# eldariont/svim-asm

Measured on AMD Instinct MI355X. Metric: CIGAR ops/sec (SV-signature extraction, human genome-genome alignment), higher is better.
Workload: dtype u32

## Files before the change

### svim_asm_amd/csrc/svx_cigar.hip

```cpp
#include "svx_internal.h"
#include "svx_postpass_dev.h"
#include "svx_segments_dev.h"

namespace {

#ifndef SVX_LANE_OPS
#define SVX_LANE_OPS 16
#endif
constexpr int kLaneOps = SVX_LANE_OPS;
constexpr int kLU = kLaneOps / 4;
constexpr int kRoundOps = 64 * kLaneOps;
#ifndef SVX_ROUNDS
#define SVX_ROUNDS 4
#endif
constexpr int kRounds = SVX_ROUNDS;
constexpr int kTileOps = kRoundOps * kRounds;
#ifndef SVX_SLAB
#define SVX_SLAB 128
#endif
constexpr int kSlab = SVX_SLAB;
#ifndef SVX_WAVES
#define SVX_WAVES 4
#endif
constexpr int kWaves = SVX_WAVES;
constexpr int kXposeU4 = 64 * kLU;
constexpr int kScanBlock = 1024;

enum { MODE_STAGE = 0, MODE_DIRECT = 1 };

struct CigarArgs {
    const uint32_t* cigar;
    const uint8_t* op;
    const uint64_t* aln_off;
    uint32_t* tile_alo;
// ... 1454 lines not shown
    a->rows = SegRowArgs{d_cigar, d_aln_off, q.d_seg_src, q.d_seg_tid, q.d_seg_pos, q.d_seg_rev, q.d_seg_qend, q.n_segs,
                         q.d_read_off, q.n_reads, q.d_segs, q.d_read_len};
    a->seg_rl = svx_ws_take<int32_t>(ctx, q.n_segs ? q.n_segs : 1);
    a->tree.segs = q.d_segs;
    a->tree.seg_rl = a->seg_rl;
    a->tree.read_len_out = q.d_read_len;
    a->tree.sorted = svx_ws_take<svx_seg>(ctx, q.n_segs ? q.n_segs : 1);
    a->tree.read_off = q.d_read_off;
    a->tree.read_len = q.d_read_len;
    a->tree.n_reads = q.n_reads;
    a->tree.o = q.params;
    a->tree.out = q.d_raw;
    svx_post_dev::PostArgs& o = a->post;
    o.raw = q.d_raw; o.read_off = q.d_read_off; o.n_reads = q.n_reads; o.contig_rank = q.d_contig_rank; o.n_contigs = q.n_contigs;
    o.min_sv = q.params.min_sv_size; o.max_sv = q.params.max_sv_size;
    o.out = q.d_post; o.out_off = q.d_post_off; o.out_cnt = q.d_post_cnt;
    o.scratch = svx_ws_take<char>(ctx, (size_t)q.n_reads * post_stride);
    o.scratch_off = nullptr;
    o.scratch_stride = post_stride;
#ifndef SVX_A3_READS_DIV
#define SVX_A3_READS_DIV 1024u
#endif
#ifndef SVX_A3_READS_MAX
#define SVX_A3_READS_MAX 32u
#endif
    const uint32_t per = q.n_reads / SVX_A3_READS_DIV;
    const uint32_t least = q.n_reads < 384u ? 1u : 2u;
    a->reads_per_block = per < least ? least : (per > SVX_A3_READS_MAX ? SVX_A3_READS_MAX : per);
    a->deal = q.n_deal_blocks ? q.d_deal : nullptr;
    a->n_deal = q.n_deal_blocks;
}

template <bool SOA>
int cigar_extract_dev_impl(svx_ctx* ctx, const uint32_t* d_cigar_or_len, const uint8_t* d_op,
                           uint64_t n_ops, const uint64_t* d_aln_off, uint32_t n_aln,
                           const int32_t* d_ref_start, uint32_t min_len, svx_sig_soa d_out,
                           uint64_t cap, uint64_t* d_n_out, const svx_a3_plan* a3 = nullptr) {
    if (!ctx || !d_n_out) return SVX_E_INVALID;
    if (n_ops >= (1ull << 32)) {
        SVX_SET_ERR(ctx, "n_ops=%llu exceeds the 2^32-1 per-call limit; split the batch",
                    (unsigned long long)n_ops);
        return SVX_E_TOO_LARGE;
    }
    SVX_HIP(ctx, hipSetDevice(ctx->device));
    if (n_ops == 0 || n_aln == 0) {
        SVX_HIP(ctx, hipMemsetAsync(d_n_out, 0, sizeof(uint64_t), ctx->stream));
        return a3 ? SVX_E_INVALID : SVX_OK;
    }
    if (!d_cigar_or_len || !d_aln_off || (SOA && !d_op)) return SVX_E_INVALID;
    if (cap > 0 && (!d_out.aln || !d_out.ref_pos || !d_out.read_pos || !d_out.len || !d_out.type))
        return SVX_E_INVALID;
    if ((reinterpret_cast<uintptr_t>(d_cigar_or_len) & 15u) ||
        (SOA && (reinterpret_cast<uintptr_t>(d_op) & 15u))) {
        SVX_SET_ERR(ctx, "device CIGAR buffers must be 16-byte aligned");
        return SVX_E_INVALID;
    }
    const bool small = n_ops <= (uint64_t)kSmallMaxTiles * kSmallTileOps && n_ops <= ctx->small_batch_ops;
    const uint32_t n_tiles = small ? (uint32_t)((n_ops + kSmallTileOps - 1) / kSmallTileOps)
                                   : (uint32_t)((n_ops + kTileOps - 1) / kTileOps);
    size_t need = svx_cigar_extract_ws_need(ctx, n_ops);
    if (a3) need += svx_take_bytes(a3->n_segs ? a3->n_segs : 1, sizeof(svx_seg)) + svx_take_bytes(a3->n_segs ? a3->n_segs : 1, 4) +
                    svx_take_bytes((size_t)a3->n_reads * a3->post_stride, 1);
    int rc = svx_ws_reserve(ctx, need);
    if (rc != SVX_OK) return rc;

    CigarArgs a;
    a.cigar = d_cigar_or_len;
    a.op = d_op;
    a.aln_off = d_aln_off;
    a.ref_start = d_ref_start;
    a.n_ops = n_ops;
    a.n_aln = n_aln;
    a.n_tiles = n_tiles;
    a.min_len = min_len;
    a.n_dense = reinterpret_cast<uint32_t*>(ctx->ws);
    a.desc = svx_ws_take<uint4>(ctx, n_tiles);
    a.desc4 = svx_ws_take<uint4>(ctx, (n_tiles + kWaves - 1) / kWaves);
    a.slab = svx_ws_take<uint4>(ctx, (size_t)n_tiles * kSlab);
    a.out_base = svx_ws_take<uint32_t>(ctx, n_tiles);
    a.carry_ref = svx_ws_take<uint32_t>(ctx, n_tiles);
    a.carry_read = svx_ws_take<uint32_t>(ctx, n_tiles);
    a.dense_list = svx_ws_take<uint32_t>(ctx, n_tiles);
    a.tile_alo = svx_ws_take<uint32_t>(ctx, n_tiles);
    const uint32_t n_scan_blocks = (n_tiles + kScanBlock - 1) / kScanBlock;
    a.blk_agg = svx_ws_take<uint4>(ctx, n_scan_blocks);
    a.blk_prefix = svx_ws_take<uint4>(ctx, n_scan_blocks);
    a.out = d_out;
    a.cap = cap;
    A3Args c;
    memset(&c, 0, sizeof(c));
    uint32_t n_a3_blocks = 0, n_post_blocks = 0;
    if (a3) {
        a3_fill(ctx, d_cigar_or_len, d_aln_off, *a3, a3->post_stride, &c);
        n_a3_blocks = c.deal ? c.n_deal : (a3->n_reads + c.reads_per_block - 1) / c.reads_per_block;
        n_post_blocks = (a3->n_reads + 255u) / 256u;
    }

    if (small) {
        rc = svx_timing_begin(ctx);
        if (rc != SVX_OK) return rc;
        rc = svx_timing_mark(ctx, 1);
        if (rc != SVX_OK) return rc;
        const uint32_t tile_blocks = (n_tiles + kWaves - 1) / kWaves;
        if (a3)
            hipLaunchKernelGGL((k_tiles_a3<SOA, kSmallTileOps, ALO_SEARCH>), dim3(n_a3_blocks + tile_blocks), dim3(64 * kWaves), 0,
                               ctx->stream, a, c, n_a3_blocks);
        else
            hipLaunchKernelGGL((k_cigar_tiles<SOA, kSmallTileOps, ALO_SEARCH>), dim3(tile_blocks), dim3(64 * kWaves), 0,
                               ctx->stream, a);
        rc = svx_timing_mark(ctx, 2);
        if (rc != SVX_OK) return rc;
        if (ctx->want_dom) {
            if (!ctx->ev_dom) SVX_HIP(ctx, hipEventCreateWithFlags(&ctx->ev_dom, hipEventDisableTiming));
            SVX_HIP(ctx, hipEventRecord(ctx->ev_dom, ctx->stream));
            ctx->ev_dom_recorded = true;
        }
#ifndef SVX_FIN_MIN_BLOCKS
#define SVX_FIN_MIN_BLOCKS 128u
#endif
        uint32_t fin_blocks = (n_tiles + kFinTiles - 1) / kFinTiles;
        if (fin_blocks < SVX_FIN_MIN_BLOCKS) fin_blocks = SVX_FIN_MIN_BLOCKS;
        if (a3)
            hipLaunchKernelGGL((k_cigar_finish_small<SOA, true>), dim3(n_post_blocks + fin_blocks), dim3(256), 0, ctx->stream, a, d_n_out,
                               c, n_post_blocks);
        else
            hipLaunchKernelGGL((k_cigar_finish_small<SOA, false>), dim3(fin_blocks), dim3(256), 0, ctx->stream, a, d_n_out, c, 0u);
        SVX_HIP(ctx, hipGetLastError());
        return svx_timing_end(ctx);
    }
    const uint32_t blocks_all = (n_tiles + kWaves - 1) / kWaves;
    const uint32_t blocks_cap = (uint32_t)ctx->n_cu * 8u;
    const uint32_t finish_blocks = (n_tiles + 256 / kFinLanes - 1) / (256 / kFinLanes);
    const uint32_t dense_blocks = n_tiles < blocks_cap ? n_tiles : blocks_cap;
    rc = svx_timing_begin(ctx);
    if (rc != SVX_OK) return rc;
    hipLaunchKernelGGL(k_tile_alo, dim3((n_aln + 255) / 256), dim3(256), 0, ctx->stream, d_aln_off, n_aln, n_tiles,
                       a.tile_alo);
    rc = svx_timing_mark(ctx, 1);
    if (rc != SVX_OK) return rc;
    hipLaunchKernelGGL((k_cigar_tiles<SOA, kTileOps, ALO_TABLE>), dim3(blocks_all), dim3(64 * kWaves), 0, ctx->stream, a);
    rc = svx_timing_mark(ctx, 2);
    if (rc != SVX_OK) return rc;
    if (ctx->want_dom) {
        if (!ctx->ev_dom) SVX_HIP(ctx, hipEventCreateWithFlags(&ctx->ev_dom, hipEventDisableTiming));
        SVX_HIP(ctx, hipEventRecord(ctx->ev_dom, ctx->stream));
        ctx->ev_dom_recorded = true;
    }
    hipLaunchKernelGGL(k_desc_scan, dim3(n_scan_blocks), dim3(kScanBlock), 0, ctx->stream, a.desc, n_tiles,
                       a.out_base, a.carry_ref, a.carry_read, a.dense_list, a.n_dense, a.blk_agg,
                       a.blk_prefix, a.n_dense + 1, d_n_out);
    if (a3) {
        hipLaunchKernelGGL(k_finish_a3, dim3(n_a3_blocks + finish_blocks), dim3(256), 0, ctx->stream, a, c, n_a3_blocks);
        hipLaunchKernelGGL((k_cigar_dense<SOA, true>), dim3(n_post_blocks + dense_blocks), dim3(64 * kWaves), 0, ctx->stream, a, c,
                           n_post_blocks);
    } else {
        hipLaunchKernelGGL(k_cigar_finish, dim3(finish_blocks), dim3(256), 0, ctx->stream, a);
        hipLaunchKernelGGL((k_cigar_dense<SOA, false>), dim3(dense_blocks), dim3(64 * kWaves), 0, ctx->stream, a, c, 0u);
    }
    SVX_HIP(ctx, hipGetLastError());
    return svx_timing_end(ctx);
}

int validate_offsets(svx_ctx* ctx, const uint64_t* aln_off, uint32_t n_aln) {
    if (n_aln == 0) return SVX_OK;
    if (!aln_off) return SVX_E_INVALID;
    if (aln_off[0] != 0) {
        SVX_SET_ERR(ctx, "aln_off[0] must be 0");
        return SVX_E_INVALID;
    }
    for (uint32_t i = 0; i < n_aln; ++i)
        if (aln_off[i + 1] < aln_off[i]) {
            SVX_SET_ERR(ctx, "aln_off must be non-decreasing (index %u)", i);
            return SVX_E_INVALID;
        }
    return SVX_OK;
}

template <bool SOA>
int cigar_extract_host_impl(svx_ctx* ctx, const uint32_t* cigar_or_len, const uint8_t* op,
                            const uint64_t* aln_off, uint32_t n_aln, const int32_t* ref_start,
                            uint32_t min_len, svx_sig_soa out, uint64_t cap, uint64_t* n_out) {
    if (!ctx || !n_out) return SVX_E_INVALID;
    *n_out = 0;
    int rc = validate_offsets(ctx, aln_off, n_aln);
    if (rc != SVX_OK) return rc;
    const uint64_t n_ops = n_aln ? aln_off[n_aln] : 0;
    if (n_ops == 0) return SVX_OK;
    if (!cigar_or_len || (SOA && !op)) return SVX_E_INVALID;
    if (n_ops >= (1ull << 32)) return SVX_E_TOO_LARGE;
    SVX_HIP(ctx, hipSetDevice(ctx->device));
    size_t need = svx_take_bytes(n_ops, 4) + (SOA ? svx_take_bytes(n_ops, 1) : 0) +
// ... 30 lines not shown
    if (m) {
        SVX_HIP(ctx, hipMemcpyAsync(out.aln, d_out.aln, m * 4, hipMemcpyDeviceToHost, ctx->stream));
        SVX_HIP(ctx, hipMemcpyAsync(out.ref_pos, d_out.ref_pos, m * 4, hipMemcpyDeviceToHost, ctx->stream));
        SVX_HIP(ctx, hipMemcpyAsync(out.read_pos, d_out.read_pos, m * 4, hipMemcpyDeviceToHost, ctx->stream));
        SVX_HIP(ctx, hipMemcpyAsync(out.len, d_out.len, m * 4, hipMemcpyDeviceToHost, ctx->stream));
        SVX_HIP(ctx, hipMemcpyAsync(out.type, d_out.type, m, hipMemcpyDeviceToHost, ctx->stream));
        SVX_HIP(ctx, hipStreamSynchronize(ctx->stream));
    }
    if (n > cap) {
        SVX_SET_ERR(ctx, "output capacity %llu < %llu signatures", (unsigned long long)cap,
                    (unsigned long long)n);
        return SVX_E_CAPACITY;
    }
    return SVX_OK;
}

}

extern "C" int svx_cigar_extract_dev(svx_ctx* ctx, const uint32_t* d_cigar, uint64_t n_ops,
                                     const uint64_t* d_aln_off, uint32_t n_aln,
                                     const int32_t* d_ref_start, uint32_t min_len, svx_sig_soa d_out,
                                     uint64_t cap, uint64_t* d_n_out) {
    return cigar_extract_dev_impl<false>(ctx, d_cigar, nullptr, n_ops, d_aln_off, n_aln, d_ref_start,
                                         min_len, d_out, cap, d_n_out);
}

int svx_cigar_extract_chain_dev(svx_ctx* ctx, const uint32_t* d_cigar, uint64_t n_ops, const uint64_t* d_aln_off, uint32_t n_aln,
                                const int32_t* d_ref_start, uint32_t min_len, svx_sig_soa d_out, uint64_t cap,
                                uint64_t* d_n_out, const svx_a3_plan* a3) {
    return cigar_extract_dev_impl<false>(ctx, d_cigar, nullptr, n_ops, d_aln_off, n_aln, d_ref_start, min_len, d_out, cap,
                                         d_n_out, a3);
}

extern "C" int svx_cigar_extract_soa_dev(svx_ctx* ctx, const uint8_t* d_op, const uint32_t* d_len,
                                         uint64_t n_ops, const uint64_t* d_aln_off, uint32_t n_aln,
                                         const int32_t* d_ref_start, uint32_t min_len,
                                         svx_sig_soa d_out, uint64_t cap, uint64_t* d_n_out) {
    return cigar_extract_dev_impl<true>(ctx, d_len, d_op, n_ops, d_aln_off, n_aln, d_ref_start,
                                        min_len, d_out, cap, d_n_out);
}

extern "C" int svx_cigar_extract(svx_ctx* ctx, const uint32_t* cigar, const uint64_t* aln_off,
                                 uint32_t n_aln, const int32_t* ref_start, uint32_t min_len,
                                 svx_sig_soa out, uint64_t cap, uint64_t* n_out) {
    return cigar_extract_host_impl<false>(ctx, cigar, nullptr, aln_off, n_aln, ref_start, min_len,
                                          out, cap, n_out);
}

extern "C" int svx_cigar_extract_soa(svx_ctx* ctx, const uint8_t* op, const uint32_t* len,
                                     const uint64_t* aln_off, uint32_t n_aln,
                                     const int32_t* ref_start, uint32_t min_len, svx_sig_soa out,
                                     uint64_t cap, uint64_t* n_out) {
    return cigar_extract_host_impl<true>(ctx, len, op, aln_off, n_aln, ref_start, min_len, out, cap,
                                         n_out);
}

extern "C" int svx_cigar_stats_dev(svx_ctx* ctx, const uint32_t* d_cigar, uint64_t n_ops,
                                   const uint64_t* d_aln_off, uint32_t n_aln, svx_aln_stats d_out) {
    if (!ctx) return SVX_E_INVALID;
    if (n_aln == 0) return SVX_OK;
    if (!d_aln_off || (n_ops && !d_cigar)) return SVX_E_INVALID;
    SVX_HIP(ctx, hipSetDevice(ctx->device));
    StatsArgs a{d_cigar, d_aln_off, n_aln, d_out};
    uint32_t blocks = (n_aln + 3) / 4;
    uint32_t cap = (uint32_t)ctx->n_cu * 8u;
    hipLaunchKernelGGL(k_cigar_stats, dim3(blocks < cap ? blocks : cap), dim3(256), 0, ctx->stream, a);
// ... 77 lines not shown
```

### svim_asm_amd/csrc/svx_collect.hip

```cpp
#include <algorithm>
#include <vector>

#include "svx_internal.h"

namespace {

struct Pack {
    size_t at = 0;
    size_t take(size_t bytes) {
        const size_t off = at;
        at = svx_align_up(at + bytes, 16);
        return off;
    }
};

int host_stage_reserve(svx_ctx* ctx, size_t bytes) {
    if (ctx->hpin_bytes >= bytes) return SVX_OK;
    if (ctx->hpin) (void)hipHostFree(ctx->hpin);
    ctx->hpin = nullptr;
    ctx->hpin_bytes = 0;
    size_t want = std::max<size_t>(bytes + bytes / 4, 1u << 20);
    void* p = nullptr;
    SVX_HIP(ctx, hipHostMalloc(&p, want, hipHostMallocDefault));
    ctx->hpin = static_cast<char*>(p);
    ctx->hpin_bytes = want;
    return SVX_OK;
}

}

extern "C" int svx_collect_batch_dev(svx_ctx* ctx, const svx_collect_dev* d) {
    if (!ctx || !d) return SVX_E_INVALID;
    if (d->n_aln == 0) {
        if (d->d_n_sig) SVX_HIP(ctx, hipMemsetAsync(d->d_n_sig, 0, 8, ctx->stream));
        return d->n_segs ? SVX_E_INVALID : SVX_OK;
    }
    if (!d->d_aln_off || !d->d_n_sig || (d->n_ops && !d->d_cigar)) return SVX_E_INVALID;
    const bool chain = d->n_reads != 0;
    if (chain && (!d->read_off || !d->d_read_off || !d->post_off || !d->d_post_off || !d->d_post_cnt || !d->d_segs ||
                  !d->d_read_len || !d->d_raw || !d->d_seg_src))
        return SVX_E_INVALID;
    if (!chain)
        return svx_cigar_extract_dev(ctx, d->d_cigar, d->n_ops, d->d_aln_off, d->n_aln, d->d_ref_start, d->min_len, d->d_sig,
                                     d->sig_cap, d->d_n_sig);
    if (!d->d_seg_tid || !d->d_seg_pos || !d->d_seg_rev || !d->d_seg_qend || (d->n_contigs && !d->d_contig_rank)) return SVX_E_INVALID;
    if ((reinterpret_cast<uintptr_t>(d->d_segs) & 7u) || (reinterpret_cast<uintptr_t>(d->d_raw) & 15u)) {
        SVX_SET_ERR(ctx, "d_segs must be 8-byte aligned and d_raw 16-byte aligned");
        return SVX_E_INVALID;
    }
    if (d->read_off[d->n_reads] != d->n_segs) return SVX_E_INVALID;
    if (d->n_chain_blocks && (!d->d_chain_deal || d->n_chain_blocks > d->n_reads || (reinterpret_cast<uintptr_t>(d->d_chain_deal) & 7u)))
        return SVX_E_INVALID;
    uint64_t stride = 0;
    int rc = svx_postpass_plan(ctx, d->read_off, d->n_reads, d->post_off, &stride);
    if (rc != SVX_OK) return rc;
    if (d->post_off[d->n_reads] && !d->d_post) return SVX_E_INVALID;
    if (stride && !ctx->split_chain && d->n_ops != 0) {
        svx_a3_plan q;
        q.d_seg_src = d->d_seg_src; q.d_seg_tid = d->d_seg_tid; q.d_seg_pos = d->d_seg_pos; q.d_seg_rev = d->d_seg_rev;
        q.d_seg_qend = d->d_seg_qend; q.n_segs = d->n_segs; q.d_read_off = d->d_read_off; q.n_reads = d->n_reads;
        q.d_contig_rank = d->d_contig_rank; q.n_contigs = d->n_contigs; q.params = d->params; q.d_segs = d->d_segs;
        q.d_read_len = d->d_read_len; q.d_raw = d->d_raw; q.d_post = d->d_post; q.d_post_off = d->d_post_off;
        q.d_post_cnt = d->d_post_cnt; q.post_stride = stride;
        q.d_deal = d->n_chain_blocks ? d->d_chain_deal : nullptr; q.n_deal_blocks = q.d_deal ? d->n_chain_blocks : 0;
        return svx_cigar_extract_chain_dev(ctx, d->d_cigar, d->n_ops, d->d_aln_off, d->n_aln, d->d_ref_start, d->min_len,
                                           d->d_sig, d->sig_cap, d->d_n_sig, &q);
    }
    rc = svx_cigar_extract_dev(ctx, d->d_cigar, d->n_ops, d->d_aln_off, d->n_aln, d->d_ref_start, d->min_len, d->d_sig,
                               d->sig_cap, d->d_n_sig);
    if (rc != SVX_OK) return rc;
    rc = svx_segments_rows_dev(ctx, d->d_cigar, d->d_aln_off, d->d_seg_src, d->d_seg_tid, d->d_seg_pos, d->d_seg_rev,
                               d->d_seg_qend, d->n_segs, d->d_read_off, d->n_reads, d->d_segs, d->d_read_len);
    if (rc != SVX_OK) return rc;
    rc = svx_segments_classify_dev(ctx, d->d_segs, d->n_segs, d->d_read_off, d->n_reads, d->d_read_len, &d->params, d->d_raw);
    if (rc != SVX_OK) return rc;
    return svx_segments_postpass_dev(ctx, d->d_raw, d->read_off, d->d_read_off, d->n_reads, d->d_contig_rank, d->n_contigs,
                                     &d->params, d->d_post, d->post_off, d->d_post_off, d->d_post_cnt);
}

static uint32_t chain_reads_per_block(uint32_t n_reads) {
    if (n_reads < 384u) return 0;
    const uint32_t per = n_reads / 1024u;
    return per < 2u ? 2u : (per > 32u ? 32u : per);
}

extern "C" int svx_chain_deal(const uint32_t* read_off, uint32_t n_reads, const uint32_t* seg_src, const uint64_t* aln_off,
                              uint32_t* deal) {
    if (!deal || (n_reads && (!read_off || !seg_src || !aln_off))) return SVX_E_INVALID;
    const uint32_t per = chain_reads_per_block(n_reads);
    if (per == 0) return 0;
    const uint32_t n_blocks = (n_reads + per - 1) / per;
    constexpr uint64_t kChunk = 128, kPerRead = 96, kPerTiny = 8;
    uint64_t total = 0;
    for (uint32_t r = 0; r < n_reads; ++r) {
        if (read_off[r + 1] < read_off[r]) return SVX_E_INVALID;
        total += kPerRead;
        for (uint32_t j = read_off[r]; j < read_off[r + 1]; ++j) {
            const uint64_t n = aln_off[(size_t)seg_src[j] + 1] - aln_off[seg_src[j]];
            total += n <= 8 ? kPerTiny : (n + kChunk - 1) / kChunk * kChunk;
        }
    }
    uint64_t prefix = 0;
    uint32_t next = 0;
    for (uint32_t r = 0; r < n_reads; ++r) {
        uint32_t b = (uint32_t)((unsigned __int128)prefix * n_blocks / total);
        if (b >= n_blocks) b = n_blocks - 1;
        for (; next <= b; ++next) { deal[2 * next] = r; deal[2 * next + 1] = read_off[r]; }
        prefix += kPerRead;
        for (uint32_t j = read_off[r]; j < read_off[r + 1]; ++j) {
            const uint64_t n = aln_off[(size_t)seg_src[j] + 1] - aln_off[seg_src[j]];
            prefix += n <= 8 ? kPerTiny : (n + kChunk - 1) / kChunk * kChunk;
        }
    }
    for (; next <= n_blocks; ++next) { deal[2 * next] = n_reads; deal[2 * next + 1] = read_off[n_reads]; }
    return (int)n_blocks;
}

extern "C" int svx_collect_batch(svx_ctx* ctx, const svx_collect_in* in, svx_collect_out* out) {
    if (!ctx || !in || !out) return SVX_E_INVALID;
    out->n_sig = 0;
    const uint32_t n_aln = in->n_aln, n_extra = in->n_extra, n_segs = in->n_segs, n_reads = in->n_reads;
    if (n_aln && (!in->aln_off || !in->ref_start)) return SVX_E_INVALID;
    if (in->n_parts && (!in->cigar_parts || !in->part_ops)) return SVX_E_INVALID;
    if (n_extra && !in->extra_off) return SVX_E_INVALID;
    if (n_segs && (!in->seg_src || !in->seg_tid || !in->seg_pos || !in->seg_rev || !in->seg_qend)) return SVX_E_INVALID;
    if (n_reads && (!in->read_off || !out->post_off || !out->post_cnt)) return SVX_E_INVALID;
    if (n_segs && !out->raw) return SVX_E_INVALID;
    if (in->n_contigs && !in->contig_rank) return SVX_E_INVALID;
    uint64_t n_ops = 0;
    for (uint32_t k = 0; k < in->n_parts; ++k) {
        if (in->part_ops[k] && !in->cigar_parts[k] && !(in->part_dev && in->part_dev[k])) return SVX_E_INVALID;
        n_ops += in->part_ops[k];
    }
    if (n_aln) {
        if (in->aln_off[0] != 0 || in->aln_off[n_aln] != n_ops) {
            SVX_SET_ERR(ctx, "aln_off must start at 0 and end at the total op count of the pools");
            return SVX_E_INVALID;
        }
        for (uint32_t i = 0; i < n_aln; ++i)
            if (in->aln_off[i + 1] < in->aln_off[i]) {
// ... 153 lines not shown
```

### svim_asm_amd/csrc/svx_internal.h

```cpp
#pragma once
#include <hip/hip_runtime.h>
#include <stdint.h>
#include <stdio.h>
#include <string.h>
#include <vector>

#include "svx.h"

struct svx_ctx {
    int device = 0;
    hipStream_t stream = nullptr;
    bool own_stream = false;
    char* ws = nullptr;
    size_t ws_bytes = 0;
    size_t ws_used = 0;
    char* stage = nullptr;
    size_t stage_bytes = 0;
    size_t stage_used = 0;
    char* hpin = nullptr;
    size_t hpin_bytes = 0;
    bool timing = false;
    hipEvent_t ev[4] = {nullptr, nullptr, nullptr, nullptr};
    bool ev_valid = false;
    hipEvent_t ev_block = nullptr;
// ... 7 lines not shown
    bool pair_lds_set = false;
    uint32_t pair_launches = 0;
    bool pair_wait_free = false;
    uint32_t pair_retries = 0;
    uint32_t pair_single_max = 131072;
    uint64_t small_batch_ops = 1ull << 23;
    bool split_chain = false;
    uint32_t link_group_min = 0;
    char err[512] = {0};
};

#define SVX_SET_ERR(ctx, ...)                                   \
    do {                                                        \
        if (ctx) snprintf((ctx)->err, sizeof((ctx)->err), __VA_ARGS__); \
    } while (0)

#define SVX_HIP(ctx, call)                                                              \
    do {                                                                                \
        hipError_t e__ = (call);                                                        \
        if (e__ != hipSuccess) {                                                        \
            SVX_SET_ERR(ctx, "%s failed: %s (%s:%d)", #call, hipGetErrorString(e__),    \
                        __FILE__, __LINE__);                                            \
            return (e__ == hipErrorOutOfMemory) ? SVX_E_NOMEM : SVX_E_HIP;              \
        }                                                                               \
    } while (0)

static inline size_t svx_align_up(size_t x, size_t a) { return (x + a - 1) / a * a; }

int svx_ws_reserve(svx_ctx* ctx, size_t total);
#define SVX_WS_BARRIER_NOTE_WORD 80
int svx_barrier_check(svx_ctx* ctx);
int svx_stage_reserve(svx_ctx* ctx, size_t total);
size_t svx_cigar_extract_ws_need(const svx_ctx* ctx, uint64_t n_ops);
size_t svx_postpass_ws_need(const uint32_t* read_off, uint32_t n_reads);

struct svx_a3_plan {
    const uint32_t* d_seg_src;
    const int32_t* d_seg_tid;
    const int32_t* d_seg_pos;
    const uint8_t* d_seg_rev;
    const int32_t* d_seg_qend;
    uint32_t n_segs;
    const uint32_t* d_read_off;
    uint32_t n_reads;
    const int32_t* d_contig_rank;
    uint32_t n_contigs;
    svx_seg_params params;
    svx_seg* d_segs;
    int32_t* d_read_len;
    svx_raw* d_raw;
    svx_post* d_post;
    const uint64_t* d_post_off;
    uint32_t* d_post_cnt;
    uint64_t post_stride;
    const uint32_t* d_deal;
    uint32_t n_deal_blocks;
};
int svx_postpass_plan(svx_ctx* ctx, const uint32_t* read_off, uint32_t n_reads, const uint64_t* out_off, uint64_t* stride);
int svx_cigar_extract_chain_dev(svx_ctx* ctx, const uint32_t* d_cigar, uint64_t n_ops, const uint64_t* d_aln_off, uint32_t n_aln,
                                const int32_t* d_ref_start, uint32_t min_len, svx_sig_soa d_out, uint64_t cap,
                                uint64_t* d_n_out, const svx_a3_plan* a3);

template <typename T>
static inline T* svx_ws_take(svx_ctx* ctx, size_t count) {
    size_t off = svx_align_up(ctx->ws_used, 256);
    ctx->ws_used = off + count * sizeof(T);
    return reinterpret_cast<T*>(ctx->ws + off);
}
template <typename T>
static inline T* svx_stage_take(svx_ctx* ctx, size_t count) {
    size_t off = svx_align_up(ctx->stage_used, 256);
    ctx->stage_used = off + count * sizeof(T);
    return reinterpret_cast<T*>(ctx->stage + off);
}
static inline size_t svx_take_bytes(size_t count, size_t elem) {
    return svx_align_up(count * elem, 256) + 256;
}

int svx_bgzf_inflate_on_stream(void* stream, const uint8_t* d_in, const uint64_t* d_in_off, const uint32_t* d_in_len,
                               const uint32_t* d_isize, const uint32_t* d_crc, uint32_t n_members, uint8_t* d_out,
                               const uint64_t* d_out_off, uint32_t* d_status, uint32_t* d_n_tok, void* d_tok, uint32_t tok_members);
uint32_t svx_bgzf_inflate_arena_members();
int svx_gather_ranges_on_stream(void* stream, const uint8_t* d_src, const uint64_t* d_src_off, const uint32_t* d_len,
                                const uint64_t* d_dst_off, uint32_t n, uint8_t* d_dst);
const uint32_t (*svx_crc32_shift_columns())[32];
int svx_wait_blocking(svx_ctx* ctx);
int svx_timing_begin(svx_ctx* ctx);
int svx_timing_mark(svx_ctx* ctx, int which);
int svx_timing_end(svx_ctx* ctx);
```

### svim_asm_amd/csrc/svx_postpass.hip

```cpp
#include "svx_internal.h"
#include "svx_postpass_dev.h"

#include <algorithm>
#include <vector>

using namespace svx_post_dev;

namespace {

constexpr int kThreads = 64;

__global__ __launch_bounds__(kThreads) void k_segments_post(PostArgs p) {
    const uint32_t r = blockIdx.x * kThreads + threadIdx.x;
    if (r < p.n_reads) post_one_read(p, r);
}

__global__ __launch_bounds__(256) void k_post_scratch_offsets(const uint32_t* read_off, uint32_t n_reads, uint64_t* scratch_off) {
    __shared__ uint64_t s_part[256];
    const uint32_t chunk = (n_reads + 255) / 256;
    const uint32_t lo = threadIdx.x * chunk, hi = min(n_reads, lo + chunk);
    uint64_t sum = 0;
    for (uint32_t r = lo; r < hi; ++r) sum += (post_scratch_bytes(read_off[r + 1] - read_off[r]) + 15) / 16 * 16;
    s_part[threadIdx.x] = sum;
    __syncthreads();
    uint64_t base = 0;
    for (uint32_t t = 0; t < threadIdx.x; ++t) base += s_part[t];
    for (uint32_t r = lo; r < hi; ++r) {
        scratch_off[r] = base;
        base += (post_scratch_bytes(read_off[r + 1] - read_off[r]) + 15) / 16 * 16;
    }
}

uint64_t post_bound(uint32_t s) { return (uint64_t)s * ((uint64_t)s + 3) / 2; }

}

extern "C" uint64_t svx_segments_postpass_bound(uint32_t n_slots) { return post_bound(n_slots); }

static uint64_t post_uniform_stride(const uint32_t* read_off, uint32_t n_reads) {
    uint32_t s_max = 0;
    for (uint32_t r = 0; r < n_reads; ++r) s_max = std::max(s_max, read_off[r + 1] - read_off[r]);
    const uint64_t stride = svx_align_up(post_scratch_bytes(s_max), 16);
    return stride * n_reads <= (64ull << 20) ? stride : 0;
}

size_t svx_postpass_ws_need(const uint32_t* read_off, uint32_t n_reads) {
    const uint64_t stride = post_uniform_stride(read_off, n_reads);
    if (stride) return svx_take_bytes((size_t)n_reads * stride, 1);
    uint64_t n_scratch = 0;
    for (uint32_t r = 0; r < n_reads; ++r) n_scratch += svx_align_up(post_scratch_bytes(read_off[r + 1] - read_off[r]), 16);
    return svx_take_bytes((size_t)n_reads + 1, 8) + svx_take_bytes(n_scratch ? n_scratch : 1, 1);
}

static int post_plan(svx_ctx* ctx, const uint32_t* read_off, uint32_t n_reads, const uint64_t* out_off,
                     std::vector<uint64_t>* scratch_off, uint64_t* n_scratch) {
    if (read_off[0] != 0) return SVX_E_INVALID;
    scratch_off->resize(n_reads);
    *n_scratch = 0;
    for (uint32_t r = 0; r < n_reads; ++r) {
        if (read_off[r + 1] < read_off[r] || out_off[r + 1] < out_off[r]) {
            SVX_SET_ERR(ctx, "read_off / out_off must be non-decreasing (index %u)", r);
            return SVX_E_INVALID;
        }
        const uint32_t s = read_off[r + 1] - read_off[r];
        if (out_off[r + 1] - out_off[r] < post_bound(s)) {
            SVX_SET_ERR(ctx, "read %u: %llu output slots for %u segment slots, svx_segments_postpass_bound() = %llu", r,
                        (unsigned long long)(out_off[r + 1] - out_off[r]), s, (unsigned long long)post_bound(s));
            return SVX_E_CAPACITY;
        }
        (*scratch_off)[r] = *n_scratch;
        *n_scratch += svx_align_up(post_scratch_bytes(s), 16);
    }
    return SVX_OK;
}

int svx_postpass_plan(svx_ctx* ctx, const uint32_t* read_off, uint32_t n_reads, const uint64_t* out_off, uint64_t* stride) {
    std::vector<uint64_t> scratch_off;
    uint64_t n_scratch = 0;
    int rc = post_plan(ctx, read_off, n_reads, out_off, &scratch_off, &n_scratch);
    if (rc != SVX_OK) return rc;
    *stride = post_uniform_stride(read_off, n_reads);
    return SVX_OK;
}

extern "C" int svx_segments_postpass_dev(svx_ctx* ctx, const svx_raw* d_raw, const uint32_t* read_off,
                                         const uint32_t* d_read_off, uint32_t n_reads, const int32_t* d_contig_rank,
                                         uint32_t n_contigs, const svx_seg_params* params, svx_post* d_out,
                                         const uint64_t* out_off, const uint64_t* d_out_off, uint32_t* d_out_cnt) {
    if (!ctx || !params) return SVX_E_INVALID;
    if (n_reads == 0) return SVX_OK;
    if (!read_off || !d_read_off || !out_off || !d_out_off || !d_out_cnt || (n_contigs && !d_contig_rank)) return SVX_E_INVALID;
    std::vector<uint64_t> scratch_off;
    uint64_t n_scratch = 0;
    int rc = post_plan(ctx, read_off, n_reads, out_off, &scratch_off, &n_scratch);
    if (rc != SVX_OK) return rc;
    if (read_off[n_reads] && (!d_raw || !d_out)) return SVX_E_INVALID;
    SVX_HIP(ctx, hipSetDevice(ctx->device));
    rc = svx_ws_reserve(ctx, svx_postpass_ws_need(read_off, n_reads));
    if (rc != SVX_OK) return rc;
    const uint64_t stride = post_uniform_stride(read_off, n_reads);
    uint64_t* d_soff = nullptr;
    char* d_scratch;
    if (stride) {
        d_scratch = svx_ws_take<char>(ctx, (size_t)n_reads * stride);
    } else {
        d_soff = svx_ws_take<uint64_t>(ctx, (size_t)n_reads + 1);
        d_scratch = svx_ws_take<char>(ctx, n_scratch ? n_scratch : 1);
        hipLaunchKernelGGL(k_post_scratch_offsets, dim3(1), dim3(256), 0, ctx->stream, d_read_off, n_reads, d_soff);
    }
    PostArgs a;
    a.scratch_stride = stride;
    a.raw = d_raw; a.read_off = d_read_off; a.n_reads = n_reads; a.contig_rank = d_contig_rank; a.n_contigs = n_contigs;
    a.min_sv = params->min_sv_size; a.max_sv = params->max_sv_size;
    a.out = d_out; a.out_off = d_out_off; a.out_cnt = d_out_cnt; a.scratch = d_scratch; a.scratch_off = d_soff;
    hipLaunchKernelGGL(k_segments_post, dim3((n_reads + kThreads - 1) / kThreads), dim3(kThreads), 0, ctx->stream, a);
    SVX_HIP(ctx, hipGetLastError());
    return SVX_OK;
}

extern "C" int svx_segments_postpass(svx_ctx* ctx, const svx_raw* raw, const uint32_t* read_off, uint32_t n_reads,
                                     const int32_t* contig_rank, uint32_t n_contigs, const svx_seg_params* params,
                                     svx_post* out, const uint64_t* out_off, uint32_t* out_cnt) {
    if (!ctx || !params) return SVX_E_INVALID;
    if (n_reads == 0) return SVX_OK;
    if (!read_off || !out_off || !out_cnt || (n_contigs && !contig_rank)) return SVX_E_INVALID;
    if (read_off[0] != 0) return SVX_E_INVALID;
    std::vector<uint64_t> scratch_off(n_reads);
    uint64_t n_scratch = 0;
    for (uint32_t r = 0; r < n_reads; ++r) {
        if (read_off[r + 1] < read_off[r] || out_off[r + 1] < out_off[r]) {
            SVX_SET_ERR(ctx, "read_off / out_off must be non-decreasing (index %u)", r);
            return SVX_E_INVALID;
        }
// ... 53 lines not shown
```

Before: 1185 billion.

## Launch CIGAR tile kernels before host postpass planning to overlap host and GPU

For large batches, the collect path now launches the tile-ALO and tile kernels first, then does the host-side postpass validation and stride planning while the GPU runs, and launches the scan/finish/dense stages afterwards. The host plan itself is rewritten as a single branch-light scan with an AVX2 variant, and the per-read scratch offset vector is dropped. The workspace is reserved up front with a conservative bound for the chain path, and a failed plan abandons the begun launch. This trades extra workspace and more complex control flow for hiding host planning latency behind GPU work.

```diff
diff --git a/svim_asm_amd/csrc/svx_cigar.hip b/svim_asm_amd/csrc/svx_cigar.hip
--- a/svim_asm_amd/csrc/svx_cigar.hip
+++ b/svim_asm_amd/csrc/svx_cigar.hip
@@ -1,5 +1,6 @@
 #include "svx_internal.h"
 #include "svx_postpass_dev.h"
+#include "svx_postplan.h"
 #include "svx_segments_dev.h"
 
 namespace {
@@ -1520,10 +1521,9 @@
 }
 
 template <bool SOA>
-int cigar_extract_dev_impl(svx_ctx* ctx, const uint32_t* d_cigar_or_len, const uint8_t* d_op,
-                           uint64_t n_ops, const uint64_t* d_aln_off, uint32_t n_aln,
-                           const int32_t* d_ref_start, uint32_t min_len, svx_sig_soa d_out,
-                           uint64_t cap, uint64_t* d_n_out, const svx_a3_plan* a3 = nullptr) {
+int cigar_check(svx_ctx* ctx, const uint32_t* d_cigar_or_len, const uint8_t* d_op, uint64_t n_ops, const uint64_t* d_aln_off,
+                uint32_t n_aln, const svx_sig_soa& d_out, uint64_t cap, uint64_t* d_n_out, bool* empty) {
+    *empty = false;
     if (!ctx || !d_n_out) return SVX_E_INVALID;
     if (n_ops >= (1ull << 32)) {
         SVX_SET_ERR(ctx, "n_ops=%llu exceeds the 2^32-1 per-call limit; split the batch",
@@ -1533,7 +1533,8 @@
     SVX_HIP(ctx, hipSetDevice(ctx->device));
     if (n_ops == 0 || n_aln == 0) {
         SVX_HIP(ctx, hipMemsetAsync(d_n_out, 0, sizeof(uint64_t), ctx->stream));
-        return a3 ? SVX_E_INVALID : SVX_OK;
+        *empty = true;
+        return SVX_OK;
     }
     if (!d_cigar_or_len || !d_aln_off || (SOA && !d_op)) return SVX_E_INVALID;
     if (cap > 0 && (!d_out.aln || !d_out.ref_pos || !d_out.read_pos || !d_out.len || !d_out.type))
@@ -1543,16 +1544,17 @@
         SVX_SET_ERR(ctx, "device CIGAR buffers must be 16-byte aligned");
         return SVX_E_INVALID;
     }
-    const bool small = n_ops <= (uint64_t)kSmallMaxTiles * kSmallTileOps && n_ops <= ctx->small_batch_ops;
-    const uint32_t n_tiles = small ? (uint32_t)((n_ops + kSmallTileOps - 1) / kSmallTileOps)
-                                   : (uint32_t)((n_ops + kTileOps - 1) / kTileOps);
-    size_t need = svx_cigar_extract_ws_need(ctx, n_ops);
-    if (a3) need += svx_take_bytes(a3->n_segs ? a3->n_segs : 1, sizeof(svx_seg)) + svx_take_bytes(a3->n_segs ? a3->n_segs : 1, 4) +
-                    svx_take_bytes((size_t)a3->n_reads * a3->post_stride, 1);
-    int rc = svx_ws_reserve(ctx, need);
-    if (rc != SVX_OK) return rc;
-
-    CigarArgs a;
+    return SVX_OK;
+}
+
+bool cigar_is_small(const svx_ctx* ctx, uint64_t n_ops) {
+    return n_ops <= (uint64_t)kSmallMaxTiles * kSmallTileOps && n_ops <= ctx->small_batch_ops;
+}
+
+void cigar_fill(svx_ctx* ctx, const uint32_t* d_cigar_or_len, const uint8_t* d_op, uint64_t n_ops, const uint64_t* d_aln_off,
+                uint32_t n_aln, const int32_t* d_ref_start, uint32_t min_len, const svx_sig_soa& d_out, uint64_t cap,
+                uint32_t n_tiles, CigarArgs* out) {
+    CigarArgs& a = *out;
     a.cigar = d_cigar_or_len;
     a.op = d_op;
     a.aln_off = d_aln_off;
@@ -1575,51 +1577,31 @@
     a.blk_prefix = svx_ws_take<uint4>(ctx, n_scan_blocks);
     a.out = d_out;
     a.cap = cap;
-    A3Args c;
-    memset(&c, 0, sizeof(c));
-    uint32_t n_a3_blocks = 0, n_post_blocks = 0;
-    if (a3) {
-        a3_fill(ctx, d_cigar_or_len, d_aln_off, *a3, a3->post_stride, &c);
-        n_a3_blocks = c.deal ? c.n_deal : (a3->n_reads + c.reads_per_block - 1) / c.reads_per_block;
-        n_post_blocks = (a3->n_reads + 255u) / 256u;
-    }
-
-    if (small) {
-        rc = svx_timing_begin(ctx);
-        if (rc != SVX_OK) return rc;
-        rc = svx_timing_mark(ctx, 1);
-        if (rc != SVX_OK) return rc;
-        const uint32_t tile_blocks = (n_tiles + kWaves - 1) / kWaves;
-        if (a3)
-            hipLaunchKernelGGL((k_tiles_a3<SOA, kSmallTileOps, ALO_SEARCH>), dim3(n_a3_blocks + tile_blocks), dim3(64 * kWaves), 0,
-                               ctx->stream, a, c, n_a3_blocks);
-        else
-            hipLaunchKernelGGL((k_cigar_tiles<SOA, kSmallTileOps, ALO_SEARCH>), dim3(tile_blocks), dim3(64 * kWaves), 0,
-                               ctx->stream, a);
-        rc = svx_timing_mark(ctx, 2);
-        if (rc != SVX_OK) return rc;
-        if (ctx->want_dom) {
-            if (!ctx->ev_dom) SVX_HIP(ctx, hipEventCreateWithFlags(&ctx->ev_dom, hipEventDisableTiming));
-            SVX_HIP(ctx, hipEventRecord(ctx->ev_dom, ctx->stream));
-            ctx->ev_dom_recorded = true;
-        }
-#ifndef SVX_FIN_MIN_BLOCKS
-#define SVX_FIN_MIN_BLOCKS 128u
-#endif
-        uint32_t fin_blocks = (n_tiles + kFinTiles - 1) / kFinTiles;
-        if (fin_blocks < SVX_FIN_MIN_BLOCKS) fin_blocks = SVX_FIN_MIN_BLOCKS;
-        if (a3)
-            hipLaunchKernelGGL((k_cigar_finish_small<SOA, true>), dim3(n_post_blocks + fin_blocks), dim3(256), 0, ctx->stream, a, d_n_out,
-                               c, n_post_blocks);
-        else
-            hipLaunchKernelGGL((k_cigar_finish_small<SOA, false>), dim3(fin_blocks), dim3(256), 0, ctx->stream, a, d_n_out, c, 0u);
-        SVX_HIP(ctx, hipGetLastError());
-        return svx_timing_end(ctx);
-    }
+}
+
+size_t a3_ws_need(const svx_a3_plan& q) {
+    return svx_take_bytes(q.n_segs ? q.n_segs : 1, sizeof(svx_seg)) + svx_take_bytes(q.n_segs ? q.n_segs : 1, 4) +
+           svx_take_bytes((size_t)q.n_reads * q.post_stride, 1);
+}
+
+struct CigarBegun {
+    CigarArgs a;
+    uint64_t* d_n_out;
+};
+static_assert(sizeof(CigarBegun) <= sizeof(svx_cigar_begun) && alignof(CigarBegun) <= alignof(svx_cigar_begun),
+              "svx_cigar_begun (svx_internal.h) must hold the begun launches' arguments");
+
+template <bool SOA>
+int cigar_stream_begin(svx_ctx* ctx, const uint32_t* d_cigar_or_len, const uint8_t* d_op, uint64_t n_ops,
+                       const uint64_t* d_aln_off, uint32_t n_aln, const int32_t* d_ref_start, uint32_t min_len,
+                       const svx_sig_soa& d_out, uint64_t cap, uint64_t* d_n_out, size_t extra_ws, CigarBegun* s) {
+    const uint32_t n_tiles = (uint32_t)((n_ops + kTileOps - 1) / kTileOps);
+    int rc = svx_ws_reserve(ctx, svx_cigar_extract_ws_need(ctx, n_ops) + extra_ws);
+    if (rc != SVX_OK) return rc;
+    cigar_fill(ctx, d_cigar_or_len, d_op, n_ops, d_aln_off, n_aln, d_ref_start, min_len, d_out, cap, n_tiles, &s->a);
+    s->d_n_out = d_n_out;
+    const CigarArgs& a = s->a;
     const uint32_t blocks_all = (n_tiles + kWaves - 1) / kWaves;
-    const uint32_t blocks_cap = (uint32_t)ctx->n_cu * 8u;
-    const uint32_t finish_blocks = (n_tiles + 256 / kFinLanes - 1) / (256 / kFinLanes);
-    const uint32_t dense_blocks = n_tiles < blocks_cap ? n_tiles : blocks_cap;
     rc = svx_timing_begin(ctx);
     if (rc != SVX_OK) return rc;
     hipLaunchKernelGGL(k_tile_alo, dim3((n_aln + 255) / 256), dim3(256), 0, ctx->stream, d_aln_off, n_aln, n_tiles,
@@ -1634,9 +1616,28 @@
         SVX_HIP(ctx, hipEventRecord(ctx->ev_dom, ctx->stream));
         ctx->ev_dom_recorded = true;
     }
+    return SVX_OK;
+}
+
+template <bool SOA>
+int cigar_stream_end(svx_ctx* ctx, const CigarBegun& s, const svx_a3_plan* a3) {
+    const CigarArgs& a = s.a;
+    const uint32_t n_tiles = a.n_tiles;
+    const uint32_t n_scan_blocks = (n_tiles + kScanBlock - 1) / kScanBlock;
+    const uint32_t blocks_cap = (uint32_t)ctx->n_cu * 8u;
+    const uint32_t finish_blocks = (n_tiles + 256 / kFinLanes - 1) / (256 / kFinLanes);
+    const uint32_t dense_blocks = n_tiles < blocks_cap ? n_tiles : blocks_cap;
+    A3Args c;
+    memset(&c, 0, sizeof(c));
+    uint32_t n_a3_blocks = 0, n_post_blocks = 0;
+    if (a3) {
+        a3_fill(ctx, a.cigar, a.aln_off, *a3, a3->post_stride, &c);
+        n_a3_blocks = c.deal ? c.n_deal : (a3->n_reads + c.reads_per_block - 1) / c.reads_per_block;
+        n_post_blocks = (a3->n_reads + 255u) / 256u;
+    }
     hipLaunchKernelGGL(k_desc_scan, dim3(n_scan_blocks), dim3(kScanBlock), 0, ctx->stream, a.desc, n_tiles,
                        a.out_base, a.carry_ref, a.carry_read, a.dense_list, a.n_dense, a.blk_agg,
-                       a.blk_prefix, a.n_dense + 1, d_n_out);
+                       a.blk_prefix, a.n_dense + 1, s.d_n_out);
     if (a3) {
         hipLaunchKernelGGL(k_finish_a3, dim3(n_a3_blocks + finish_blocks), dim3(256), 0, ctx->stream, a, c, n_a3_blocks);
         hipLaunchKernelGGL((k_cigar_dense<SOA, true>), dim3(n_post_blocks + dense_blocks), dim3(64 * kWaves), 0, ctx->stream, a, c,
@@ -1645,6 +1646,67 @@
         hipLaunchKernelGGL(k_cigar_finish, dim3(finish_blocks), dim3(256), 0, ctx->stream, a);
         hipLaunchKernelGGL((k_cigar_dense<SOA, false>), dim3(dense_blocks), dim3(64 * kWaves), 0, ctx->stream, a, c, 0u);
     }
+    SVX_HIP(ctx, hipGetLastError());
+    return svx_timing_end(ctx);
+}
+
+template <bool SOA>
+int cigar_extract_dev_impl(svx_ctx* ctx, const uint32_t* d_cigar_or_len, const uint8_t* d_op,
+                           uint64_t n_ops, const uint64_t* d_aln_off, uint32_t n_aln,
+                           const int32_t* d_ref_start, uint32_t min_len, svx_sig_soa d_out,
+                           uint64_t cap, uint64_t* d_n_out, const svx_a3_plan* a3 = nullptr) {
+    bool empty = false;
+    int rc = cigar_check<SOA>(ctx, d_cigar_or_len, d_op, n_ops, d_aln_off, n_aln, d_out, cap, d_n_out, &empty);
+    if (rc != SVX_OK) return rc;
+    if (empty) return a3 ? SVX_E_INVALID : SVX_OK;
+    if (!cigar_is_small(ctx, n_ops)) {
+        CigarBegun s;
+        rc = cigar_stream_begin<SOA>(ctx, d_cigar_or_len, d_op, n_ops, d_aln_off, n_aln, d_ref_start, min_len, d_out, cap,
+                                     d_n_out, a3 ? a3_ws_need(*a3) : 0, &s);
+        if (rc != SVX_OK) return rc;
+        return cigar_stream_end<SOA>(ctx, s, a3);
+    }
+    const uint32_t n_tiles = (uint32_t)((n_ops + kSmallTileOps - 1) / kSmallTileOps);
+    rc = svx_ws_reserve(ctx, svx_cigar_extract_ws_need(ctx, n_ops) + (a3 ? a3_ws_need(*a3) : 0));
+    if (rc != SVX_OK) return rc;
+    CigarArgs a;
+    cigar_fill(ctx, d_cigar_or_len, d_op, n_ops, d_aln_off, n_aln, d_ref_start, min_len, d_out, cap, n_tiles, &a);
+    A3Args c;
+    memset(&c, 0, sizeof(c));
+    uint32_t n_a3_blocks = 0, n_post_blocks = 0;
+    if (a3) {
+        a3_fill(ctx, d_cigar_or_len, d_aln_off, *a3, a3->post_stride, &c);
+        n_a3_blocks = c.deal ? c.n_deal : (a3->n_reads + c.reads_per_block - 1) / c.reads_per_block;
+        n_post_blocks = (a3->n_reads + 255u) / 256u;
+    }
+    rc = svx_timing_begin(ctx);
+    if (rc != SVX_OK) return rc;
+    rc = svx_timing_mark(ctx, 1);
+    if (rc != SVX_OK) return rc;
+    const uint32_t tile_blocks = (n_tiles + kWaves - 1) / kWaves;
+    if (a3)
+        hipLaunchKernelGGL((k_tiles_a3<SOA, kSmallTileOps, ALO_SEARCH>), dim3(n_a3_blocks + tile_blocks), dim3(64 * kWaves), 0,
+                           ctx->stream, a, c, n_a3_blocks);
+    else
+        hipLaunchKernelGGL((k_cigar_tiles<SOA, kSmallTileOps, ALO_SEARCH>), dim3(tile_blocks), dim3(64 * kWaves), 0,
+                           ctx->stream, a);
+    rc = svx_timing_mark(ctx, 2);
+    if (rc != SVX_OK) return rc;
+    if (ctx->want_dom) {
+        if (!ctx->ev_dom) SVX_HIP(ctx, hipEventCreateWithFlags(&ctx->ev_dom, hipEventDisableTiming));
+        SVX_HIP(ctx, hipEventRecord(ctx->ev_dom, ctx->stream));
+        ctx->ev_dom_recorded = true;
+    }
+#ifndef SVX_FIN_MIN_BLOCKS
+#define SVX_FIN_MIN_BLOCKS 128u
+#endif
+    uint32_t fin_blocks = (n_tiles + kFinTiles - 1) / kFinTiles;
+    if (fin_blocks < SVX_FIN_MIN_BLOCKS) fin_blocks = SVX_FIN_MIN_BLOCKS;
+    if (a3)
+        hipLaunchKernelGGL((k_cigar_finish_small<SOA, true>), dim3(n_post_blocks + fin_blocks), dim3(256), 0, ctx->stream, a, d_n_out,
+                           c, n_post_blocks);
+    else
+        hipLaunchKernelGGL((k_cigar_finish_small<SOA, false>), dim3(fin_blocks), dim3(256), 0, ctx->stream, a, d_n_out, c, 0u);
     SVX_HIP(ctx, hipGetLastError());
     return svx_timing_end(ctx);
 }
@@ -1741,6 +1803,30 @@
                                          d_n_out, a3);
 }
 
+bool svx_cigar_is_streaming(const svx_ctx* ctx, uint64_t n_ops) { return n_ops != 0 && !cigar_is_small(ctx, n_ops); }
+
+size_t svx_cigar_chain_ws_bound(uint32_t n_segs) {
+    return svx_take_bytes(n_segs ? n_segs : 1, sizeof(svx_seg)) + svx_take_bytes(n_segs ? n_segs : 1, 4) +
+           svx_take_bytes(kSvxPostUniformMax, 1);
+}
+
+int svx_cigar_stream_begin_dev(svx_ctx* ctx, const uint32_t* d_cigar, uint64_t n_ops, const uint64_t* d_aln_off, uint32_t n_aln,
+                               const int32_t* d_ref_start, uint32_t min_len, svx_sig_soa d_out, uint64_t cap,
+                               uint64_t* d_n_out, size_t extra_ws, svx_cigar_begun* st) {
+    bool empty = false;
+    int rc = cigar_check<false>(ctx, d_cigar, nullptr, n_ops, d_aln_off, n_aln, d_out, cap, d_n_out, &empty);
+    if (rc != SVX_OK) return rc;
+    if (empty || cigar_is_small(ctx, n_ops)) return SVX_E_INVALID;
+    return cigar_stream_begin<false>(ctx, d_cigar, nullptr, n_ops, d_aln_off, n_aln, d_ref_start, min_len, d_out, cap, d_n_out,
+                                     extra_ws, reinterpret_cast<CigarBegun*>(st));
+}
+
+int svx_cigar_stream_end_dev(svx_ctx* ctx, const svx_cigar_begun* st, const svx_a3_plan* a3) {
+    return cigar_stream_end<false>(ctx, *reinterpret_cast<const CigarBegun*>(st), a3);
+}
+
+void svx_cigar_stream_abandon(svx_ctx* ctx, const svx_cigar_begun*) { ctx->ev_valid = false; }
+
 extern "C" int svx_cigar_extract_soa_dev(svx_ctx* ctx, const uint8_t* d_op, const uint32_t* d_len,
                                          uint64_t n_ops, const uint64_t* d_aln_off, uint32_t n_aln,
                                          const int32_t* d_ref_start, uint32_t min_len,
diff --git a/svim_asm_amd/csrc/svx_collect.hip b/svim_asm_amd/csrc/svx_collect.hip
--- a/svim_asm_amd/csrc/svx_collect.hip
+++ b/svim_asm_amd/csrc/svx_collect.hip
@@ -51,10 +51,21 @@
     if (d->read_off[d->n_reads] != d->n_segs) return SVX_E_INVALID;
     if (d->n_chain_blocks && (!d->d_chain_deal || d->n_chain_blocks > d->n_reads || (reinterpret_cast<uintptr_t>(d->d_chain_deal) & 7u)))
         return SVX_E_INVALID;
+    const bool begun = svx_cigar_is_streaming(ctx, d->n_ops);
+    svx_cigar_begun st;
+    int rc = SVX_OK;
+    if (begun) {
+        rc = svx_cigar_stream_begin_dev(ctx, d->d_cigar, d->n_ops, d->d_aln_off, d->n_aln, d->d_ref_start, d->min_len, d->d_sig,
+                                        d->sig_cap, d->d_n_sig, svx_cigar_chain_ws_bound(d->n_segs), &st);
+        if (rc != SVX_OK) return rc;
+    }
     uint64_t stride = 0;
-    int rc = svx_postpass_plan(ctx, d->read_off, d->n_reads, d->post_off, &stride);
-    if (rc != SVX_OK) return rc;
-    if (d->post_off[d->n_reads] && !d->d_post) return SVX_E_INVALID;
+    rc = svx_postpass_plan(ctx, d->read_off, d->n_reads, d->post_off, &stride);
+    if (rc == SVX_OK && d->post_off[d->n_reads] && !d->d_post) rc = SVX_E_INVALID;
+    if (rc != SVX_OK) {
+        if (begun) svx_cigar_stream_abandon(ctx, &st);
+        return rc;
+    }
     if (stride && !ctx->split_chain && d->n_ops != 0) {
         svx_a3_plan q;
         q.d_seg_src = d->d_seg_src; q.d_seg_tid = d->d_seg_tid; q.d_seg_pos = d->d_seg_pos; q.d_seg_rev = d->d_seg_rev;
@@ -63,11 +74,13 @@
         q.d_read_len = d->d_read_len; q.d_raw = d->d_raw; q.d_post = d->d_post; q.d_post_off = d->d_post_off;
         q.d_post_cnt = d->d_post_cnt; q.post_stride = stride;
         q.d_deal = d->n_chain_blocks ? d->d_chain_deal : nullptr; q.n_deal_blocks = q.d_deal ? d->n_chain_blocks : 0;
+        if (begun) return svx_cigar_stream_end_dev(ctx, &st, &q);
         return svx_cigar_extract_chain_dev(ctx, d->d_cigar, d->n_ops, d->d_aln_off, d->n_aln, d->d_ref_start, d->min_len,
                                            d->d_sig, d->sig_cap, d->d_n_sig, &q);
     }
-    rc = svx_cigar_extract_dev(ctx, d->d_cigar, d->n_ops, d->d_aln_off, d->n_aln, d->d_ref_start, d->min_len, d->d_sig,
-                               d->sig_cap, d->d_n_sig);
+    rc = begun ? svx_cigar_stream_end_dev(ctx, &st, nullptr)
+               : svx_cigar_extract_dev(ctx, d->d_cigar, d->n_ops, d->d_aln_off, d->n_aln, d->d_ref_start, d->min_len, d->d_sig,
+                                       d->sig_cap, d->d_n_sig);
     if (rc != SVX_OK) return rc;
     rc = svx_segments_rows_dev(ctx, d->d_cigar, d->d_aln_off, d->d_seg_src, d->d_seg_tid, d->d_seg_pos, d->d_seg_rev,
                                d->d_seg_qend, d->n_segs, d->d_read_off, d->n_reads, d->d_segs, d->d_read_len);
@@ -103,9 +116,8 @@
     uint64_t prefix = 0;
     uint32_t next = 0;
     for (uint32_t r = 0; r < n_reads; ++r) {
-        uint32_t b = (uint32_t)((unsigned __int128)prefix * n_blocks / total);
-        if (b >= n_blocks) b = n_blocks - 1;
-        for (; next <= b; ++next) { deal[2 * next] = r; deal[2 * next + 1] = read_off[r]; }
+        const unsigned __int128 at = (unsigned __int128)prefix * n_blocks;
+        for (; next < n_blocks && (unsigned __int128)next * total <= at; ++next) { deal[2 * next] = r; deal[2 * next + 1] = read_off[r]; }
         prefix += kPerRead;
         for (uint32_t j = read_off[r]; j < read_off[r + 1]; ++j) {
             const uint64_t n = aln_off[(size_t)seg_src[j] + 1] - aln_off[seg_src[j]];
diff --git a/svim_asm_amd/csrc/svx_internal.h b/svim_asm_amd/csrc/svx_internal.h
--- a/svim_asm_amd/csrc/svx_internal.h
+++ b/svim_asm_amd/csrc/svx_internal.h
@@ -63,7 +63,7 @@
 int svx_barrier_check(svx_ctx* ctx);
 int svx_stage_reserve(svx_ctx* ctx, size_t total);
 size_t svx_cigar_extract_ws_need(const svx_ctx* ctx, uint64_t n_ops);
-size_t svx_postpass_ws_need(const uint32_t* read_off, uint32_t n_reads);
+size_t svx_postpass_ws_need(const uint32_t* read_off, uint32_t n_reads, uint64_t stride, uint64_t* n_scratch);
 
 struct svx_a3_plan {
     const uint32_t* d_seg_src;
@@ -92,6 +92,15 @@
                                 const int32_t* d_ref_start, uint32_t min_len, svx_sig_soa d_out, uint64_t cap,
                                 uint64_t* d_n_out, const svx_a3_plan* a3);
 
+struct svx_cigar_begun { alignas(16) unsigned char args[256]; };
+bool svx_cigar_is_streaming(const svx_ctx* ctx, uint64_t n_ops);
+size_t svx_cigar_chain_ws_bound(uint32_t n_segs);
+int svx_cigar_stream_begin_dev(svx_ctx* ctx, const uint32_t* d_cigar, uint64_t n_ops, const uint64_t* d_aln_off, uint32_t n_aln,
+                               const int32_t* d_ref_start, uint32_t min_len, svx_sig_soa d_out, uint64_t cap,
+                               uint64_t* d_n_out, size_t extra_ws, svx_cigar_begun* st);
+int svx_cigar_stream_end_dev(svx_ctx* ctx, const svx_cigar_begun* st, const svx_a3_plan* a3);
+void svx_cigar_stream_abandon(svx_ctx* ctx, const svx_cigar_begun* st);
+
 template <typename T>
 static inline T* svx_ws_take(svx_ctx* ctx, size_t count) {
     size_t off = svx_align_up(ctx->ws_used, 256);
diff --git a/svim_asm_amd/csrc/svx_postpass.hip b/svim_asm_amd/csrc/svx_postpass.hip
--- a/svim_asm_amd/csrc/svx_postpass.hip
+++ b/svim_asm_amd/csrc/svx_postpass.hip
@@ -1,5 +1,6 @@
 #include "svx_internal.h"
 #include "svx_postpass_dev.h"
+#include "svx_postplan.h"
 
 #include <algorithm>
 #include <vector>
@@ -37,50 +38,30 @@
 
 extern "C" uint64_t svx_segments_postpass_bound(uint32_t n_slots) { return post_bound(n_slots); }
 
-static uint64_t post_uniform_stride(const uint32_t* read_off, uint32_t n_reads) {
-    uint32_t s_max = 0;
-    for (uint32_t r = 0; r < n_reads; ++r) s_max = std::max(s_max, read_off[r + 1] - read_off[r]);
-    const uint64_t stride = svx_align_up(post_scratch_bytes(s_max), 16);
-    return stride * n_reads <= (64ull << 20) ? stride : 0;
+static size_t post_slice_bytes(uint32_t s) { return post_scratch_bytes(s); }
+
+static uint64_t post_scratch_total(const uint32_t* read_off, uint32_t n_reads) {
+    uint64_t n_scratch = 0;
+    for (uint32_t r = 0; r < n_reads; ++r) n_scratch += svx_align_up(post_scratch_bytes(read_off[r + 1] - read_off[r]), 16);
+    return n_scratch;
 }
 
-size_t svx_postpass_ws_need(const uint32_t* read_off, uint32_t n_reads) {
-    const uint64_t stride = post_uniform_stride(read_off, n_reads);
+size_t svx_postpass_ws_need(const uint32_t* read_off, uint32_t n_reads, uint64_t stride, uint64_t* n_scratch) {
     if (stride) return svx_take_bytes((size_t)n_reads * stride, 1);
-    uint64_t n_scratch = 0;
-    for (uint32_t r = 0; r < n_reads; ++r) n_scratch += svx_align_up(post_scratch_bytes(read_off[r + 1] - read_off[r]), 16);
-    return svx_take_bytes((size_t)n_reads + 1, 8) + svx_take_bytes(n_scratch ? n_scratch : 1, 1);
-}
-
-static int post_plan(svx_ctx* ctx, const uint32_t* read_off, uint32_t n_reads, const uint64_t* out_off,
-                     std::vector<uint64_t>* scratch_off, uint64_t* n_scratch) {
-    if (read_off[0] != 0) return SVX_E_INVALID;
-    scratch_off->resize(n_reads);
-    *n_scratch = 0;
-    for (uint32_t r = 0; r < n_reads; ++r) {
-        if (read_off[r + 1] < read_off[r] || out_off[r + 1] < out_off[r]) {
-            SVX_SET_ERR(ctx, "read_off / out_off must be non-decreasing (index %u)", r);
-            return SVX_E_INVALID;
-        }
-        const uint32_t s = read_off[r + 1] - read_off[r];
-        if (out_off[r + 1] - out_off[r] < post_bound(s)) {
-            SVX_SET_ERR(ctx, "read %u: %llu output slots for %u segment slots, svx_segments_postpass_bound() = %llu", r,
-                        (unsigned long long)(out_off[r + 1] - out_off[r]), s, (unsigned long long)post_bound(s));
-            return SVX_E_CAPACITY;
-        }
-        (*scratch_off)[r] = *n_scratch;
-        *n_scratch += svx_align_up(post_scratch_bytes(s), 16);
-    }
-    return SVX_OK;
+    *n_scratch = post_scratch_total(read_off, n_reads);
+    return svx_take_bytes((size_t)n_reads + 1, 8) + svx_take_bytes(*n_scratch ? *n_scratch : 1, 1);
 }
 
 int svx_postpass_plan(svx_ctx* ctx, const uint32_t* read_off, uint32_t n_reads, const uint64_t* out_off, uint64_t* stride) {
-    std::vector<uint64_t> scratch_off;
-    uint64_t n_scratch = 0;
-    int rc = post_plan(ctx, read_off, n_reads, out_off, &scratch_off, &n_scratch);
-    if (rc != SVX_OK) return rc;
-    *stride = post_uniform_stride(read_off, n_reads);
-    return SVX_OK;
+    uint32_t r = 0;
+    const int rc = svx_postplan(read_off, n_reads, out_off, post_slice_bytes, stride, &r);
+    if (rc == SVX_E_INVALID && r != ~0u) SVX_SET_ERR(ctx, "read_off / out_off must be non-decreasing (index %u)", r);
+    if (rc == SVX_E_CAPACITY) {
+        const uint32_t s = read_off[r + 1] - read_off[r];
+        SVX_SET_ERR(ctx, "read %u: %llu output slots for %u segment slots, svx_segments_postpass_bound() = %llu", r,
+                    (unsigned long long)(out_off[r + 1] - out_off[r]), s, (unsigned long long)post_bound(s));
+    }
+    return rc;
 }
 
 extern "C" int svx_segments_postpass_dev(svx_ctx* ctx, const svx_raw* d_raw, const uint32_t* read_off,
@@ -90,15 +71,13 @@
     if (!ctx || !params) return SVX_E_INVALID;
     if (n_reads == 0) return SVX_OK;
     if (!read_off || !d_read_off || !out_off || !d_out_off || !d_out_cnt || (n_contigs && !d_contig_rank)) return SVX_E_INVALID;
-    std::vector<uint64_t> scratch_off;
-    uint64_t n_scratch = 0;
-    int rc = post_plan(ctx, read_off, n_reads, out_off, &scratch_off, &n_scratch);
+    uint64_t stride = 0, n_scratch = 0;
+    int rc = svx_postpass_plan(ctx, read_off, n_reads, out_off, &stride);
     if (rc != SVX_OK) return rc;
     if (read_off[n_reads] && (!d_raw || !d_out)) return SVX_E_INVALID;
     SVX_HIP(ctx, hipSetDevice(ctx->device));
-    rc = svx_ws_reserve(ctx, svx_postpass_ws_need(read_off, n_reads));
+    rc = svx_ws_reserve(ctx, svx_postpass_ws_need(read_off, n_reads, stride, &n_scratch));
     if (rc != SVX_OK) return rc;
-    const uint64_t stride = post_uniform_stride(read_off, n_reads);
     uint64_t* d_soff = nullptr;
     char* d_scratch;
     if (stride) {
diff --git a/svim_asm_amd/csrc/svx_postplan.h b/svim_asm_amd/csrc/svx_postplan.h
--- /dev/null
+++ b/svim_asm_amd/csrc/svx_postplan.h
@@ -0,0 +1,60 @@
+#pragma once
+#include <stddef.h>
+#include <stdint.h>
+
+#include "svx.h"
+
+static inline uint64_t svx_postplan_bound(uint32_t s) { return (uint64_t)s * ((uint64_t)s + 3) / 2; }
+
+constexpr uint64_t kSvxPostUniformMax = 64ull << 20;
+
+struct svx_postplan_scan_t { uint64_t doubt; uint32_t s_max; };
+static inline __attribute__((always_inline)) svx_postplan_scan_t svx_postplan_scan(const uint32_t* read_off, uint32_t n_reads,
+                                                                                  const uint64_t* out_off) {
+    uint64_t doubt = 0;
+    uint32_t s_max = 0;
+    for (uint32_t r = 0; r < n_reads; ++r) {
+        const uint32_t a = read_off[r], b = read_off[r + 1], s = b - a;
+        const uint64_t oa = out_off[r], ob = out_off[r + 1], d = ob - oa;
+        const uint64_t bound = ((uint64_t)s * s + 3 * (uint64_t)s) >> 1;
+        doubt |= ((uint64_t)b - (uint64_t)a) | oa | ob | d | (d - bound);
+        s_max = s > s_max ? s : s_max;
+    }
+    return svx_postplan_scan_t{doubt, s_max};
+}
+#if defined(__x86_64__) && (defined(__GNUC__) || defined(__clang__))
+__attribute__((target("avx2"))) static inline svx_postplan_scan_t svx_postplan_scan_avx2(const uint32_t* read_off, uint32_t n_reads,
+                                                                                          const uint64_t* out_off) {
+    return svx_postplan_scan(read_off, n_reads, out_off);
+}
+static inline bool svx_postplan_has_wide() { return __builtin_cpu_supports("avx2") != 0; }
+#else
+static inline svx_postplan_scan_t svx_postplan_scan_avx2(const uint32_t* read_off, uint32_t n_reads, const uint64_t* out_off) {
+    return svx_postplan_scan(read_off, n_reads, out_off);
+}
+static inline bool svx_postplan_has_wide() { return false; }
+#endif
+static inline svx_postplan_scan_t svx_postplan_scan_base(const uint32_t* read_off, uint32_t n_reads, const uint64_t* out_off) {
+    return svx_postplan_scan(read_off, n_reads, out_off);
+}
+
+static inline int svx_postplan_with(bool wide, const uint32_t* read_off, uint32_t n_reads, const uint64_t* out_off,
+                                    size_t (*slice_bytes)(uint32_t slots), uint64_t* stride, uint32_t* bad) {
+    *stride = 0;
+    *bad = ~0u;
+    if (read_off[0] != 0) return SVX_E_INVALID;
+    const svx_postplan_scan_t q = wide ? svx_postplan_scan_avx2(read_off, n_reads, out_off) : svx_postplan_scan_base(read_off, n_reads, out_off);
+    if (q.doubt >> 63) {
+        for (uint32_t r = 0; r < n_reads; ++r) {
+            if (read_off[r + 1] < read_off[r] || out_off[r + 1] < out_off[r]) { *bad = r; return SVX_E_INVALID; }
+            if (out_off[r + 1] - out_off[r] < svx_postplan_bound(read_off[r + 1] - read_off[r])) { *bad = r; return SVX_E_CAPACITY; }
+        }
+    }
+    const uint64_t one = ((uint64_t)slice_bytes(q.s_max) + 15) / 16 * 16;
+    *stride = one * n_reads <= kSvxPostUniformMax ? one : 0;
+    return SVX_OK;
+}
+static inline int svx_postplan(const uint32_t* read_off, uint32_t n_reads, const uint64_t* out_off,
+                               size_t (*slice_bytes)(uint32_t slots), uint64_t* stride, uint32_t* bad) {
+    return svx_postplan_with(svx_postplan_has_wide(), read_off, n_reads, out_off, slice_bytes, stride, bad);
+}
```

Result: no change. 1177 billion (median of 2 runs) (-0.7%).
